# google-research/hyperbo

Measured on AMD Instinct MI355X. Metric: GP NLL+grad evals/sec at N=8192 D=16 fp64, higher is better.
Workload: dtype f64

## Files before the change

### hyperbo_amd/csrc/chol.hip

```cpp
#include "hbo_internal.h"
#include <type_traits>
#include <limits.h>
#include <string.h>

namespace {

#include "panel_dev.h"
#ifdef HBO_POTF2_TIMING
__device__ unsigned long long hbo_dbg_stamps[64];
__device__ unsigned long long hbo_dbg_wall[3 * 256];
__device__ unsigned long long hbo_dbg_trsm[3 * 128];
__device__ int hbo_dbg_trsm_panel = 36;
#define STAMP(i) do { if (threadIdx.x == 0) hbo_dbg_stamps[i] = __builtin_readcyclecounter(); } while (0)
#else
#define STAMP(i) do {} while (0)
#endif
#ifndef HBO_POTF2_WAVES
#define HBO_POTF2_WAVES 8
#endif
constexpr int POTF2_WAVES = HBO_POTF2_WAVES;
constexpr int POTF2_THREADS = 64 * POTF2_WAVES;
template <typename T>
__device__ __forceinline__ void potf2_body(const TaskDesc& t, int p, int* info_slot, unsigned char* smem) {
  typedef typename Mma<T>::acc_t acc_t;
  T* sT = reinterpret_cast<T*>(smem);
  T* sM = sT + 36 * TILE_ELEMS;
  T* sDinv = sM + TILE_ELEMS;
  const int64_t ld = t.ld;
  T* Ab = static_cast<T*>(t.A) + (int64_t)p * NB * ld + (int64_t)p * NB;
  T* Wb = static_cast<T*>(t.W) + (int64_t)p * NB * ld + (int64_t)p * NB;
  const int tid = threadIdx.x, lane = tid & 63, wave = tid >> 6;
  const int l15 = lane & 15, lq = lane >> 4;
  const int ei = (tid & 255) >> 4, ej = tid & 15;
  STAMP(0);
#ifdef HBO_POTF2_TIMING
  if (tid == 0 && blockIdx.x == 0 && p < 256) {
    hbo_dbg_wall[3 * p] = wall_clock64();
    hbo_dbg_wall[3 * p + 2] = ((unsigned long long)__builtin_amdgcn_s_getreg((20 << 0) | (0 << 6) | (31 << 11)) << 32) |
                              (unsigned)__builtin_amdgcn_s_getreg((4 << 0) | (0 << 6) | (31 << 11));
  }
#endif

  auto factor_leaf = [&](int jb, const acc_t* from_regs = nullptr) {
    T* dt = sT + tri_index(jb, jb) * TILE_ELEMS;
    acc_t acc;
    if (from_regs) acc = *from_regs;
    else {
#pragma unroll
      for (int r = 0; r < 4; ++r) acc[r] = dt[Mma<T>::crow(lane, r) * TS + l15];
    }
    const int bad = leaf_cholesky4<T>(acc, dt, sM, sDinv + jb * 16, Wb + (int64_t)(jb * 16) * ld + jb * 16, ld, lane);
    if (bad >= 0 && lane == 0) atomicMin(info_slot, p * NB + jb * 16 + bad + 1);
  };
  auto solve_tile = [&](int jb, int R) {
    T* xt = sT + tri_index(R, jb) * TILE_ELEMS;
    acc_t acc = {0, 0, 0, 0};
#pragma unroll
    for (int kk = 0; kk < 4; ++kk) acc = Mma<T>::mma(xt[l15 * TS + kk * 4 + lq], sM[l15 * TS + kk * 4 + lq], acc);
#pragma unroll
    for (int r = 0; r < 4; ++r) xt[Mma<T>::crow(lane, r) * TS + l15] = acc[r];
  };
  auto update_tile = [&](int jb, int I, int J) {
    T* ct = sT + tri_index(I, J) * TILE_ELEMS;
    const T* at = sT + tri_index(I, jb) * TILE_ELEMS;
    const T* bt = sT + tri_index(J, jb) * TILE_ELEMS;
    acc_t acc;
#pragma unroll
    for (int r = 0; r < 4; ++r) acc[r] = ct[Mma<T>::crow(lane, r) * TS + l15];
#pragma unroll
    for (int kk = 0; kk < 4; ++kk) acc = Mma<T>::mma(-at[l15 * TS + kk * 4 + lq], bt[l15 * TS + kk * 4 + lq], acc);
#pragma unroll
    for (int r = 0; r < 4; ++r) ct[Mma<T>::crow(lane, r) * TS + l15] = acc[r];
  };

  auto update_tile2 = [&](int jb, int I0, int J0, int I1, int J1) {
    T* c0 = sT + tri_index(I0, J0) * TILE_ELEMS;
    T* c1 = sT + tri_index(I1, J1) * TILE_ELEMS;
    const T* a0 = sT + tri_index(I0, jb) * TILE_ELEMS;
    const T* b0 = sT + tri_index(J0, jb) * TILE_ELEMS;
    const T* a1 = sT + tri_index(I1, jb) * TILE_ELEMS;
    const T* b1 = sT + tri_index(J1, jb) * TILE_ELEMS;
    acc_t x0, x1;
    T fa0[4], fb0[4], fa1[4], fb1[4];
#pragma unroll
    for (int r = 0; r < 4; ++r) { x0[r] = c0[Mma<T>::crow(lane, r) * TS + l15]; x1[r] = c1[Mma<T>::crow(lane, r) * TS + l15]; }
#pragma unroll
    for (int kk = 0; kk < 4; ++kk) {
      fa0[kk] = -a0[l15 * TS + kk * 4 + lq]; fb0[kk] = b0[l15 * TS + kk * 4 + lq];
      fa1[kk] = -a1[l15 * TS + kk * 4 + lq]; fb1[kk] = b1[l15 * TS + kk * 4 + lq];
    }
#pragma unroll
    for (int kk = 0; kk < 4; ++kk) { x0 = Mma<T>::mma(fa0[kk], fb0[kk], x0); x1 = Mma<T>::mma(fa1[kk], fb1[kk], x1); }
#pragma unroll
    for (int r = 0; r < 4; ++r) { c0[Mma<T>::crow(lane, r) * TS + l15] = x0[r]; c1[Mma<T>::crow(lane, r) * TS + l15] = x1[r]; }
  };

  int nleaf = 8;
  {
    const int64_t rows = (int64_t)t.n - (int64_t)p * NB;
    if (rows < NB) nleaf = rows <= 0 ? 0 : (int)((rows + 15) / 16);
    for (int jb = nleaf + wave; jb < 8; jb += POTF2_WAVES)
#pragma unroll
      for (int r = 0; r < 4; ++r) {
        const int row = Mma<T>::crow(lane, r);
        gst(Wb + (int64_t)(jb * 16 + row) * ld + jb * 16 + l15, row == l15 ? (T)1 : (T)0);
      }
    if (tid < NB && tid >= nleaf * 16) sDinv[tid] = (T)1;
  }
  const bool lead_tile0 = nleaf > 0;
  acc_t tile0 = {0, 0, 0, 0};
  if (wave == 0 && lead_tile0) {
#pragma unroll
    for (int r = 0; r < 4; ++r) {
      const int row = Mma<T>::crow(lane, r);
      const int rr = row > l15 ? row : l15, cc = row > l15 ? l15 : row;
      tile0[r] = gld(Ab + (int64_t)rr * ld + cc);
    }
  }
  constexpr int NSH = POTF2_THREADS / 256;
  const int sh = __builtin_amdgcn_readfirstlane(tid >> 8);
  T vload[36 / NSH];
  auto load_issue = [&](auto share) {
    constexpr int SH = decltype(share)::value;
    int tile = 0;
#pragma unroll
    for (int I = 0; I < 8; ++I)
#pragma unroll
      for (int J = 0; J <= I; ++J, ++tile) {
        if (tile % NSH != SH) continue;
        if (tile == 0 && lead_tile0) { vload[0] = (T)0; continue; }
        int r = ei, c = ej;
        if (I == J && ej > ei) { r = ej; c = ei; }
        vload[tile / NSH] = gld(Ab + (int64_t)(I * 16 + r) * ld + J * 16 + c);
      }
  };
  auto load_commit = [&](auto share) {
    constexpr int SH = decltype(share)::value;
#pragma unroll
    for (int k = 0; k < 36 / NSH; ++k)
      if (!(k == 0 && SH == 0 && lead_tile0)) sT[(k * NSH + SH) * TILE_ELEMS + ei * TS + ej] = vload[k];
  };
  static_assert(NSH == 1 || NSH == 2, "one or two 256-thread groups");
  if (NSH == 1 || sh == 0) load_issue(std::integral_constant<int, 0>());
  else load_issue(std::integral_constant<int, NSH - 1>());
  if (wave == 0 && lead_tile0) factor_leaf(0, &tile0);
  if (NSH == 1 || sh == 0) load_commit(std::integral_constant<int, 0>());
  else load_commit(std::integral_constant<int, NSH - 1>());
  STAMP(1);
  __syncthreads();
  STAMP(2);
  for (int jb = 0; jb < nleaf; ++jb) {
    for (int R = jb + 1 + wave; R < nleaf; R += POTF2_WAVES) solve_tile(jb, R);
    __syncthreads();
    STAMP(3 + 3 * jb);
    if (jb == nleaf - 1) break;
    {
      const int m = nleaf - 1 - jb;
      const int ntiles = m * (m + 1) / 2;
      constexpr int NH = POTF2_WAVES == 8 ? 6 : POTF2_WAVES - 1;
      const int hw = POTF2_WAVES == 8 ? (wave < 4 ? wave : wave - 1) : wave;
      const int n0 = (ntiles - 1 > 4 * NH + 1) ? (ntiles - 1 - (4 * NH + 1)) / POTF2_WAVES : 0;
      const int nshared = ntiles - n0;
      auto tile_of = [&](int tix, int& I, int& J) {
        int ii = 0;
        while ((ii + 1) * (ii + 2) / 2 <= tix) ++ii;
        I = jb + 1 + ii; J = jb + 1 + tix - ii * (ii + 1) / 2;
      };
      if (wave == 0) {
        update_tile(jb, jb + 1, jb + 1);
        factor_leaf(jb + 1);
        STAMP(4 + 3 * jb);
        for (int tix = nshared; tix < ntiles; ++tix) { int I, J; tile_of(tix, I, J); update_tile(jb, I, J); }
      } else if (!(POTF2_WAVES == 8 && wave == 4)) {
        int tix = hw;
        for (; tix + NH < nshared; tix += 2 * NH) {
          int I0, J0, I1, J1;
          tile_of(tix, I0, J0); tile_of(tix + NH, I1, J1);
          update_tile2(jb, I0, J0, I1, J1);
        }
        if (tix < nshared) { int I, J; tile_of(tix, I, J); update_tile(jb, I, J); }
      }
    }
    __syncthreads();
    STAMP(5 + 3 * jb);
  }
  STAMP(30);

  auto store_share = [&](auto share) {
    constexpr int SH = decltype(share)::value;
    int tile = 0;
#pragma unroll
    for (int I = 0; I < 8; ++I)
#pragma unroll
      for (int J = 0; J <= I; ++J, ++tile) {
        if (tile % NSH != SH) continue;
        T v = sT[tile * TILE_ELEMS + ei * TS + ej];
        if (I == J && ej > ei) v = (T)0;
        gst(Ab + (int64_t)(I * 16 + ei) * ld + J * 16 + ej, v);
      }
  };
  if (NSH == 1 || sh == 0) store_share(std::integral_constant<int, 0>());
  else store_share(std::integral_constant<int, NSH - 1>());
  STAMP(31);
  STAMP(32);
#ifdef HBO_POTF2_TIMING
  if (tid == 0 && blockIdx.x == 0 && p < 256) hbo_dbg_wall[3 * p + 1] = wall_clock64();
#endif
}
template <typename T>
__global__ __launch_bounds__(POTF2_THREADS) void potf2_kernel(const TaskDesc* tasks, int p, int* info, int* yield_flag, unsigned long long* tl) {
  extern __shared__ __attribute__((aligned(16))) unsigned char smem[];
  __builtin_amdgcn_s_setprio(3);
  const TaskDesc& t = tasks[blockIdx.x];
  if (p >= t.nblk) return;
  tl_begin(tl);
  int tok = 0;
  if (yield_flag && threadIdx.x == 0) tok = yield_enter(yield_flag);
  potf2_body<T>(t, p, info + blockIdx.x, smem);
  if (yield_flag) {
    __syncthreads();
    if (threadIdx.x == 0) yield_leave(yield_flag, tok);
  }
  tl_end(tl);
}

template <typename T>
constexpr int trsm_tile() { return sizeof(T) == 8 ? 256 : TILE_ELEMS; }
template <typename T>
__device__ __forceinline__ int trsm_at(int r, int c) { return sizeof(T) == 8 ? r * 16 + (c ^ ((r >> 1) << 1)) : r * TS + c; }
template <typename T>
constexpr int trsm_lds_bytes() { return (28 + 8 + 4) * trsm_tile<T>() * (int)sizeof(T); }
__device__ __forceinline__ int strict_index(int I, int J) { return I * (I - 1) / 2 + J; }

template <typename T, bool IDENT>
__device__ __forceinline__ void trsm_body(const TaskDesc& t, int p, int64_t row0, unsigned char* smem, bool stage) {
  typedef typename Mma<T>::acc_t acc_t;
  constexpr int TE = trsm_tile<T>();
  T* sLt = reinterpret_cast<T*>(smem);
  T* sWi = sLt + 28 * TE;
  T* sSc = sWi + 8 * TE;
  const int64_t ld = t.ld;
  const int tid = threadIdx.x, lane = tid & 63, wave = tid >> 6;
  const int l15 = lane & 15, lq = lane >> 4;
  const T* Lb = static_cast<const T*>(t.A) + (int64_t)p * NB * ld + (int64_t)p * NB;
  const T* Wb = static_cast<const T*>(t.W) + (int64_t)p * NB * ld + (int64_t)p * NB;

  const int64_t wrow0 = row0 + wave * 16;
  const int rg = IDENT ? (int)((wrow0 - (int64_t)p * NB) >> 4) : 0;
  T* Ap = IDENT ? nullptr : static_cast<T*>(t.A) + wrow0 * ld + (int64_t)p * NB;
  T* Wout = IDENT ? static_cast<T*>(t.W) + (int64_t)p * NB * ld + (int64_t)p * NB : nullptr;

  acc_t areg[8];
#pragma unroll
  for (int jb = 0; jb < 8; ++jb)
#pragma unroll
    for (int r = 0; r < 4; ++r) {
      const int row = Mma<T>::crow(lane, r);
      if (IDENT) areg[jb][r] = (rg == jb && row == l15) ? (T)1 : (T)0;
      else areg[jb][r] = gld(Ap + (int64_t)row * ld + jb * 16 + l15);
    }
  if (stage) {
    const int i = tid >> 4, j = tid & 15;
    int tile = 0;
#pragma unroll
    for (int I = 1; I < 8; ++I)
#pragma unroll
      for (int J = 0; J < I; ++J, ++tile)
        sLt[tile * TE + trsm_at<T>(i, j)] = gld(Lb + (int64_t)(I * 16 + i) * ld + J * 16 + j);
#pragma unroll
    for (int b = 0; b < 8; ++b)
      sWi[b * TE + trsm_at<T>(i, j)] = gld(Wb + (int64_t)(b * 16 + i) * ld + b * 16 + j);
  }
  if (stage) __syncthreads();

  T* sc = sSc + wave * TE;
  T xneg[8][4];
#pragma unroll
  for (int jb = 0; jb < 8; ++jb) {
    acc_t acc = areg[jb];
    acc_t acc2 = (acc_t){0, 0, 0, 0};
#pragma unroll
    for (int kb = 0; kb < 8; ++kb) {
      if (kb < jb) {
        const T* lt = sLt + strict_index(jb, kb) * TE;
#pragma unroll
        for (int kk = 0; kk < 4; ++kk) {
          const T bfrag = lt[trsm_at<T>(l15, kk * 4 + lq)];
          if (kb & 1) acc2 = Mma<T>::mma(xneg[kb][kk], bfrag, acc2);
          else acc = Mma<T>::mma(xneg[kb][kk], bfrag, acc);
        }
      }
    }
#pragma unroll
    for (int r = 0; r < 4; ++r) acc[r] += acc2[r];
    __builtin_amdgcn_wave_barrier();
#pragma unroll
    for (int r = 0; r < 4; ++r) sc[trsm_at<T>(Mma<T>::crow(lane, r), l15)] = acc[r];
    __builtin_amdgcn_wave_barrier();
    T ta[4];
#pragma unroll
    for (int kk = 0; kk < 4; ++kk) ta[kk] = sc[trsm_at<T>(l15, kk * 4 + lq)];
    acc_t x = (acc_t){0, 0, 0, 0};
    const T* wt = sWi + jb * TE;
#pragma unroll
    for (int kk = 0; kk < 4; ++kk) {
      const T bfrag = wt[trsm_at<T>(l15, kk * 4 + lq)];
      x = Mma<T>::mma(ta[kk], bfrag, x);
    }
#pragma unroll
    for (int r = 0; r < 4; ++r) {
      const int row = Mma<T>::crow(lane, r);
      if (IDENT) {
        if (rg != jb) gst(Wout + (int64_t)(jb * 16 + l15) * ld + rg * 16 + row, x[r]);
      } else {
        gst(Ap + (int64_t)row * ld + jb * 16 + l15, x[r]);
      }
    }
    if (jb < 7) {
      __builtin_amdgcn_wave_barrier();
#pragma unroll
      for (int r = 0; r < 4; ++r) sc[trsm_at<T>(Mma<T>::crow(lane, r), l15)] = x[r];
      __builtin_amdgcn_wave_barrier();
#pragma unroll
      for (int kk = 0; kk < 4; ++kk) xneg[jb][kk] = -sc[trsm_at<T>(l15, kk * 4 + lq)];
    }
  }
}
template <typename T, bool IDENT>
__global__ __launch_bounds__(256) void trsm_kernel(const TaskDesc* tasks, int p_arg, int* yield_tab, unsigned long long* tl) {
  extern __shared__ __attribute__((aligned(16))) unsigned char smem[];
  __builtin_amdgcn_s_setprio(3);
  const TaskDesc& t = tasks[blockIdx.z];
  const int p = IDENT ? p_arg + (int)blockIdx.y : p_arg;
  if (p >= t.nblk) return;
#ifdef HBO_POTF2_TIMING
  const bool dbg = !IDENT && p == hbo_dbg_trsm_panel && blockIdx.x < 128 && threadIdx.x == 0;
  if (dbg) {
    hbo_dbg_trsm[3 * blockIdx.x] = wall_clock64();
    hbo_dbg_trsm[3 * blockIdx.x + 2] = ((unsigned long long)__builtin_amdgcn_s_getreg((20 << 0) | (0 << 6) | (31 << 11)) << 32) |
                                       (unsigned)__builtin_amdgcn_s_getreg((4 << 0) | (0 << 6) | (31 << 11));
  }
#endif
  int64_t row0;
  if (IDENT) {
    row0 = (int64_t)p * NB + (int64_t)blockIdx.x * 64;
  } else {
    const int64_t first = (int64_t)(p + 1) * NB;
    const int64_t nrows = (int64_t)(t.nblk + 1) * NB - first;
    const int64_t bx = ((int64_t)blockIdx.x + 3 * (int64_t)blockIdx.z) % gridDim.x;
    if (bx * 64 >= nrows) return;
    row0 = first + bx * 64;
  }
  int tok = 0;
  tl_begin(tl);
  if (yield_tab && threadIdx.x == 0) tok = yield_enter(yield_tab);
  trsm_body<T, IDENT>(t, p, row0, smem, true);
  if (yield_tab) {
    __syncthreads();
    if (threadIdx.x == 0) yield_leave(yield_tab, tok);
  }
  tl_end(tl);
#ifdef HBO_POTF2_TIMING
  if (dbg) hbo_dbg_trsm[3 * blockIdx.x + 1] = wall_clock64();
#endif
}

template <typename T>
void set_attrs() {
  static unsigned long long seen = 0;
  if (!hbo_first_use_on_device(seen)) return;
  hipFuncSetAttribute(reinterpret_cast<const void*>(&potf2_kernel<T>),
                      hipFuncAttributeMaxDynamicSharedMemorySize, potf2_lds_bytes<T>());
  hipFuncSetAttribute(reinterpret_cast<const void*>(&trsm_kernel<T, false>),
                      hipFuncAttributeMaxDynamicSharedMemorySize, trsm_lds_bytes<T>());
  hipFuncSetAttribute(reinterpret_cast<const void*>(&trsm_kernel<T, true>),
                      hipFuncAttributeMaxDynamicSharedMemorySize, trsm_lds_bytes<T>());
}

template <typename T>
void potf2_t(const TaskDesc* tasks, int ntasks, int p, int* info, hipStream_t st, int* yield_flag, unsigned long long* tl) {
  set_attrs<T>();
  hipLaunchKernelGGL((potf2_kernel<T>), dim3(ntasks), dim3(POTF2_THREADS), potf2_lds_bytes<T>(), st, tasks, p, info,
                     yield_flag, tl);
}
template <typename T>
void trsm_t(const TaskDesc* tasks, int ntasks, int p, int max_nblk, hipStream_t st, int* yield_tab, unsigned long long* tl) {
  set_attrs<T>();
  const int nrows = (max_nblk + 1 - (p + 1)) * NB;
  if (nrows <= 0) return;
  hipLaunchKernelGGL((trsm_kernel<T, false>), dim3(nrows / 64, 1, ntasks), dim3(256), trsm_lds_bytes<T>(), st,
                     tasks, p, yield_tab, tl);
}
template <typename T>
void trtri_diag_t(const TaskDesc* tasks, int ntasks, int p_lo, int p_hi, hipStream_t st) {
  set_attrs<T>();
  if (p_hi <= p_lo) return;
  hipLaunchKernelGGL((trsm_kernel<T, true>), dim3(2, p_hi - p_lo, ntasks), dim3(256), trsm_lds_bytes<T>(), st,
                     tasks, p_lo, (int*)nullptr, (unsigned long long*)nullptr);
}

}

#ifdef HBO_POTF2_TIMING
void dbg_read_stamps(unsigned long long* host) { hipMemcpyFromSymbol(host, HIP_SYMBOL(hbo_dbg_stamps), sizeof(unsigned long long) * 64); }
extern "C" void hbo_dbg_trsm_wall(unsigned long long* host, int panel) {
  if (host) hipMemcpyFromSymbol(host, HIP_SYMBOL(hbo_dbg_trsm), sizeof(unsigned long long) * 3 * 128);
  else hipMemcpyToSymbol(HIP_SYMBOL(hbo_dbg_trsm_panel), &panel, sizeof(int));
}
extern "C" void hbo_dbg_potf2_wall(unsigned long long* host) { hipMemcpyFromSymbol(host, HIP_SYMBOL(hbo_dbg_wall), sizeof(unsigned long long) * 3 * 256); }
#endif
void launch_potf2(int dtype, const TaskDesc* tasks, int ntasks, int p, int* info, hipStream_t st, int* yield_flag, unsigned long long* tl) {
  if (dtype == HBO_F64) potf2_t<double>(tasks, ntasks, p, info, st, yield_flag, tl);
  else potf2_t<float>(tasks, ntasks, p, info, st, yield_flag, tl);
}
void launch_trsm(int dtype, const TaskDesc* tasks, int ntasks, int p, int max_nblk, hipStream_t st, int* yield_tab, unsigned long long* tl) {
  if (dtype == HBO_F64) trsm_t<double>(tasks, ntasks, p, max_nblk, st, yield_tab, tl);
  else trsm_t<float>(tasks, ntasks, p, max_nblk, st, yield_tab, tl);
}
void launch_trtri_diag(int dtype, const TaskDesc* tasks, int ntasks, int p_lo, int p_hi, hipStream_t st) {
  if (dtype == HBO_F64) trtri_diag_t<double>(tasks, ntasks, p_lo, p_hi, st);
  else trtri_diag_t<float>(tasks, ntasks, p_lo, p_hi, st);
}
```

Baseline: 93.31.

## Rework potf2 loads/stores and trsm operand layout to remove LDS transposes

The potf2 panel loads now use paired vector loads with symmetric diagonal fill. The next diagonal tile is factored straight from registers. Finished columns are written to global memory by an otherwise idle wave during the update phase, so the final store only writes the remaining tiles. The trsm kernel changes its fragment layout so solve results feed the next MMA directly from registers, which drops the per-wave scratch LDS round trips and wave barriers. It also adds a configurable wave count and occupancy hint. These changes risk subtle layout and indexing errors and add more register pressure.

```diff
diff --git a/hyperbo_amd/csrc/chol.hip b/hyperbo_amd/csrc/chol.hip
--- a/hyperbo_amd/csrc/chol.hip
+++ b/hyperbo_amd/csrc/chol.hip
@@ -73,6 +73,31 @@
     for (int r = 0; r < 4; ++r) ct[Mma<T>::crow(lane, r) * TS + l15] = acc[r];
   };
 
+  auto update_tile_regs = [&](int jb, int I, int J) -> acc_t {
+    const T* ct = sT + tri_index(I, J) * TILE_ELEMS;
+    const T* at = sT + tri_index(I, jb) * TILE_ELEMS;
+    const T* bt = sT + tri_index(J, jb) * TILE_ELEMS;
+    acc_t acc;
+#pragma unroll
+    for (int r = 0; r < 4; ++r) acc[r] = ct[Mma<T>::crow(lane, r) * TS + l15];
+#pragma unroll
+    for (int kk = 0; kk < 4; ++kk) acc = Mma<T>::mma(-at[l15 * TS + kk * 4 + lq], bt[l15 * TS + kk * 4 + lq], acc);
+    return acc;
+  };
+  auto store_column = [&](int jb, int nl) {
+#pragma unroll 2
+    for (int R = jb; R < nl; ++R) {
+      const T* tt = sT + tri_index(R, jb) * TILE_ELEMS;
+#pragma unroll
+      for (int q = 0; q < 4; ++q) {
+        const int row = 4 * q + lq;
+        T v = tt[row * TS + l15];
+        if (R == jb && l15 > row) v = (T)0;
+        gst(Ab + (int64_t)(R * 16 + row) * ld + jb * 16 + l15, v);
+      }
+    }
+  };
+
   auto update_tile2 = [&](int jb, int I0, int J0, int I1, int J1) {
     T* c0 = sT + tri_index(I0, J0) * TILE_ELEMS;
     T* c1 = sT + tri_index(I1, J1) * TILE_ELEMS;
@@ -119,33 +144,53 @@
   }
   constexpr int NSH = POTF2_THREADS / 256;
   const int sh = __builtin_amdgcn_readfirstlane(tid >> 8);
-  T vload[36 / NSH];
-  auto load_issue = [&](auto share) {
-    constexpr int SH = decltype(share)::value;
+  constexpr int NG = POTF2_THREADS / 128;
+  const int grp = __builtin_amdgcn_readfirstlane(tid >> 7);
+  const int pr = (tid & 127) >> 3, pc = (tid & 7) * 2;
+  typedef T pair_t __attribute__((ext_vector_type(2), aligned(sizeof(T))));
+  pair_t vload[(36 + NG - 1) / NG];
+  auto load_issue = [&](auto group) {
+    constexpr int G = decltype(group)::value;
     int tile = 0;
 #pragma unroll
     for (int I = 0; I < 8; ++I)
 #pragma unroll
       for (int J = 0; J <= I; ++J, ++tile) {
-        if (tile % NSH != SH) continue;
-        if (tile == 0 && lead_tile0) { vload[0] = (T)0; continue; }
-        int r = ei, c = ej;
-        if (I == J && ej > ei) { r = ej; c = ei; }
-        vload[tile / NSH] = gld(Ab + (int64_t)(I * 16 + r) * ld + J * 16 + c);
-      }
-  };
-  auto load_commit = [&](auto share) {
-    constexpr int SH = decltype(share)::value;
-#pragma unroll
-    for (int k = 0; k < 36 / NSH; ++k)
-      if (!(k == 0 && SH == 0 && lead_tile0)) sT[(k * NSH + SH) * TILE_ELEMS + ei * TS + ej] = vload[k];
+        if (tile % NG != G) continue;
+        if (tile == 0 && lead_tile0) { vload[0] = (pair_t){(T)0, (T)0}; continue; }
+        vload[tile / NG] = *(const HBO_GLOBAL pair_t*)(Ab + (int64_t)(I * 16 + pr) * ld + J * 16 + pc);
+      }
+  };
+  auto load_commit = [&](auto group) {
+    constexpr int G = decltype(group)::value;
+    int tile = 0;
+#pragma unroll
+    for (int I = 0; I < 8; ++I)
+#pragma unroll
+      for (int J = 0; J <= I; ++J, ++tile) {
+        if (tile % NG != G) continue;
+        if (tile == 0 && lead_tile0) continue;
+        T* tt = sT + tile * TILE_ELEMS;
+        const pair_t v = vload[tile / NG];
+        if (I == J) {
+          if (pc <= pr) { tt[pr * TS + pc] = v[0]; tt[pc * TS + pr] = v[0]; }
+          if (pc + 1 <= pr) { tt[pr * TS + pc + 1] = v[1]; tt[(pc + 1) * TS + pr] = v[1]; }
+        } else {
+          tt[pr * TS + pc] = v[0]; tt[pr * TS + pc + 1] = v[1];
+        }
+      }
   };
   static_assert(NSH == 1 || NSH == 2, "one or two 256-thread groups");
-  if (NSH == 1 || sh == 0) load_issue(std::integral_constant<int, 0>());
-  else load_issue(std::integral_constant<int, NSH - 1>());
+  static_assert(NG == 2 || NG == 4, "two or four 128-thread groups");
+  auto by_group = [&](auto f) {
+    if (grp == 0) f(std::integral_constant<int, 0>());
+    else if (grp == 1) f(std::integral_constant<int, 1>());
+    else if (NG == 4 && grp == 2) f(std::integral_constant<int, 2 % NG>());
+    else f(std::integral_constant<int, NG - 1>());
+  };
+  by_group(load_issue);
   if (wave == 0 && lead_tile0) factor_leaf(0, &tile0);
-  if (NSH == 1 || sh == 0) load_commit(std::integral_constant<int, 0>());
-  else load_commit(std::integral_constant<int, NSH - 1>());
+  by_group(load_commit);
   STAMP(1);
   __syncthreads();
   STAMP(2);
@@ -167,11 +212,14 @@
         I = jb + 1 + ii; J = jb + 1 + tix - ii * (ii + 1) / 2;
       };
       if (wave == 0) {
-        update_tile(jb, jb + 1, jb + 1);
-        factor_leaf(jb + 1);
+        const acc_t next_diag = update_tile_regs(jb, jb + 1, jb + 1);
+        factor_leaf(jb + 1, &next_diag);
         STAMP(4 + 3 * jb);
         for (int tix = nshared; tix < ntiles; ++tix) { int I, J; tile_of(tix, I, J); update_tile(jb, I, J); }
-      } else if (!(POTF2_WAVES == 8 && wave == 4)) {
+      } else if (POTF2_WAVES == 8 && wave == 4) {
+        store_column(jb, nleaf);
+      } else {
+        if (POTF2_WAVES != 8 && wave == POTF2_WAVES - 1) store_column(jb, nleaf);
         int tix = hw;
         for (; tix + NH < nshared; tix += 2 * NH) {
           int I0, J0, I1, J1;
@@ -194,12 +242,15 @@
 #pragma unroll
       for (int J = 0; J <= I; ++J, ++tile) {
         if (tile % NSH != SH) continue;
+        if (J < nleaf - 1 && I < nleaf) continue;
         T v = sT[tile * TILE_ELEMS + ei * TS + ej];
         if (I == J && ej > ei) v = (T)0;
         gst(Ab + (int64_t)(I * 16 + ei) * ld + J * 16 + ej, v);
       }
   };
-  if (NSH == 1 || sh == 0) store_share(std::integral_constant<int, 0>());
+  if (nleaf == 8) {
+    if (tid < 256) gst(Ab + (int64_t)(7 * 16 + ei) * ld + 7 * 16 + ej, ej > ei ? (T)0 : sT[35 * TILE_ELEMS + ei * TS + ej]);
+  } else if (NSH == 1 || sh == 0) store_share(std::integral_constant<int, 0>());
   else store_share(std::integral_constant<int, NSH - 1>());
   STAMP(31);
   STAMP(32);
@@ -224,12 +275,25 @@
   tl_end(tl);
 }
 
-template <typename T>
-constexpr int trsm_tile() { return sizeof(T) == 8 ? 256 : TILE_ELEMS; }
-template <typename T>
-__device__ __forceinline__ int trsm_at(int r, int c) { return sizeof(T) == 8 ? r * 16 + (c ^ ((r >> 1) << 1)) : r * TS + c; }
-template <typename T>
-constexpr int trsm_lds_bytes() { return (28 + 8 + 4) * trsm_tile<T>() * (int)sizeof(T); }
+#ifndef HBO_TRSM_WAVES
+#define HBO_TRSM_WAVES 4
+#endif
+constexpr int TRSM_WAVES = HBO_TRSM_WAVES;
+constexpr int TRSM_THREADS = 64 * TRSM_WAVES;
+constexpr int TRSM_ROWS = 16 * TRSM_WAVES;
+static_assert(TRSM_WAVES == 4 || TRSM_WAVES == 8, "one or two 256-thread groups; NB rows are a whole number of workgroups");
+template <typename T>
+constexpr int trsm_tile() { return 256; }
+template <typename T>
+__device__ __forceinline__ int trsm_kcol(int lq, int r) { return sizeof(T) == 8 ? 2 * lq + (r & 1) + 8 * (r >> 1) : lq + 4 * r; }
+template <typename T>
+__device__ __forceinline__ int trsm_arow(int i) { return sizeof(T) == 8 ? 2 * (i & 3) + ((i >> 2) & 1) + (i & 8) : (i >> 2) + 4 * (i & 3); }
+template <typename T>
+__device__ __forceinline__ int trsm_at(int r, int c) {
+  return sizeof(T) == 8 ? r * 16 + (c ^ ((r & 12) | ((r & 1) << 1) | ((r >> 1) & 1))) : r * 16 + (c ^ r);
+}
+template <typename T>
+constexpr int trsm_lds_bytes() { return (28 + 8) * trsm_tile<T>() * (int)sizeof(T); }
 __device__ __forceinline__ int strict_index(int I, int J) { return I * (I - 1) / 2 + J; }
 
 template <typename T, bool IDENT>
@@ -238,96 +302,87 @@
   constexpr int TE = trsm_tile<T>();
   T* sLt = reinterpret_cast<T*>(smem);
   T* sWi = sLt + 28 * TE;
-  T* sSc = sWi + 8 * TE;
   const int64_t ld = t.ld;
   const int tid = threadIdx.x, lane = tid & 63, wave = tid >> 6;
   const int l15 = lane & 15, lq = lane >> 4;
+  const int ar = trsm_arow<T>(l15);
   const T* Lb = static_cast<const T*>(t.A) + (int64_t)p * NB * ld + (int64_t)p * NB;
   const T* Wb = static_cast<const T*>(t.W) + (int64_t)p * NB * ld + (int64_t)p * NB;
 
   const int64_t wrow0 = row0 + wave * 16;
   const int rg = IDENT ? (int)((wrow0 - (int64_t)p * NB) >> 4) : 0;
-  T* Ap = IDENT ? nullptr : static_cast<T*>(t.A) + wrow0 * ld + (int64_t)p * NB;
+  T* Ap = IDENT ? nullptr : static_cast<T*>(t.A) + (wrow0 + l15) * ld + (int64_t)p * NB;
   T* Wout = IDENT ? static_cast<T*>(t.W) + (int64_t)p * NB * ld + (int64_t)p * NB : nullptr;
 
-  acc_t areg[8];
+  acc_t y[8];
 #pragma unroll
   for (int jb = 0; jb < 8; ++jb)
 #pragma unroll
     for (int r = 0; r < 4; ++r) {
-      const int row = Mma<T>::crow(lane, r);
-      if (IDENT) areg[jb][r] = (rg == jb && row == l15) ? (T)1 : (T)0;
-      else areg[jb][r] = gld(Ap + (int64_t)row * ld + jb * 16 + l15);
+      const int k = trsm_kcol<T>(lq, r);
+      if (IDENT) y[jb][r] = (rg == jb && k == l15) ? (T)1 : (T)0;
+      else y[jb][r] = gld(Ap + jb * 16 + k);
     }
   if (stage) {
-    const int i = tid >> 4, j = tid & 15;
-    int tile = 0;
-#pragma unroll
-    for (int I = 1; I < 8; ++I)
-#pragma unroll
-      for (int J = 0; J < I; ++J, ++tile)
-        sLt[tile * TE + trsm_at<T>(i, j)] = gld(Lb + (int64_t)(I * 16 + i) * ld + J * 16 + j);
-#pragma unroll
-    for (int b = 0; b < 8; ++b)
-      sWi[b * TE + trsm_at<T>(i, j)] = gld(Wb + (int64_t)(b * 16 + i) * ld + b * 16 + j);
-  }
-  if (stage) __syncthreads();
-
-  T* sc = sSc + wave * TE;
-  T xneg[8][4];
+    constexpr int NSH = TRSM_THREADS / 256;
+    const int i = (tid & 255) >> 4, j = tid & 15;
+    auto stage_share = [&](auto share) {
+      constexpr int SH = decltype(share)::value;
+      T v[36 / NSH];
+      int tile = 0;
+#pragma unroll
+      for (int I = 1; I < 8; ++I)
+#pragma unroll
+        for (int J = 0; J < I; ++J, ++tile)
+          if (tile % NSH == SH) v[tile / NSH] = gld(Lb + (int64_t)(I * 16 + i) * ld + J * 16 + j);
+#pragma unroll
+      for (int b = 0; b < 8; ++b)
+        if ((28 + b) % NSH == SH) v[(28 + b) / NSH] = gld(Wb + (int64_t)(b * 16 + i) * ld + b * 16 + j);
+#pragma unroll
+      for (int q = 0; q < 36 / NSH; ++q) sLt[(q * NSH + SH) * TE + trsm_at<T>(i, j)] = v[q];
+    };
+    if (NSH == 1 || __builtin_amdgcn_readfirstlane(tid >> 8) == 0) stage_share(std::integral_constant<int, 0>());
+    else stage_share(std::integral_constant<int, NSH - 1>());
+    __syncthreads();
+  }
+
 #pragma unroll
   for (int jb = 0; jb < 8; ++jb) {
-    acc_t acc = areg[jb];
+    acc_t acc = y[jb];
     acc_t acc2 = (acc_t){0, 0, 0, 0};
 #pragma unroll
     for (int kb = 0; kb < 8; ++kb) {
       if (kb < jb) {
         const T* lt = sLt + strict_index(jb, kb) * TE;
 #pragma unroll
-        for (int kk = 0; kk < 4; ++kk) {
-          const T bfrag = lt[trsm_at<T>(l15, kk * 4 + lq)];
-          if (kb & 1) acc2 = Mma<T>::mma(xneg[kb][kk], bfrag, acc2);
-          else acc = Mma<T>::mma(xneg[kb][kk], bfrag, acc);
+        for (int r = 0; r < 4; ++r) {
+          const T afrag = lt[trsm_at<T>(ar, trsm_kcol<T>(lq, r))];
+          if (kb & 1) acc2 = Mma<T>::mma(afrag, y[kb][r], acc2);
+          else acc = Mma<T>::mma(afrag, y[kb][r], acc);
         }
       }
     }
 #pragma unroll
     for (int r = 0; r < 4; ++r) acc[r] += acc2[r];
-    __builtin_amdgcn_wave_barrier();
-#pragma unroll
-    for (int r = 0; r < 4; ++r) sc[trsm_at<T>(Mma<T>::crow(lane, r), l15)] = acc[r];
-    __builtin_amdgcn_wave_barrier();
-    T ta[4];
-#pragma unroll
-    for (int kk = 0; kk < 4; ++kk) ta[kk] = sc[trsm_at<T>(l15, kk * 4 + lq)];
     acc_t x = (acc_t){0, 0, 0, 0};
     const T* wt = sWi + jb * TE;
 #pragma unroll
-    for (int kk = 0; kk < 4; ++kk) {
-      const T bfrag = wt[trsm_at<T>(l15, kk * 4 + lq)];
-      x = Mma<T>::mma(ta[kk], bfrag, x);
-    }
+    for (int r = 0; r < 4; ++r) x = Mma<T>::mma(wt[trsm_at<T>(ar, trsm_kcol<T>(lq, r))], acc[r], x);
 #pragma unroll
     for (int r = 0; r < 4; ++r) {
-      const int row = Mma<T>::crow(lane, r);
+      const int k = trsm_kcol<T>(lq, r);
       if (IDENT) {
-        if (rg != jb) gst(Wout + (int64_t)(jb * 16 + l15) * ld + rg * 16 + row, x[r]);
+        if (rg != jb) gst(Wout + (int64_t)(jb * 16 + k) * ld + rg * 16 + l15, x[r]);
       } else {
-        gst(Ap + (int64_t)row * ld + jb * 16 + l15, x[r]);
-      }
-    }
-    if (jb < 7) {
-      __builtin_amdgcn_wave_barrier();
-#pragma unroll
-      for (int r = 0; r < 4; ++r) sc[trsm_at<T>(Mma<T>::crow(lane, r), l15)] = x[r];
-      __builtin_amdgcn_wave_barrier();
-#pragma unroll
-      for (int kk = 0; kk < 4; ++kk) xneg[jb][kk] = -sc[trsm_at<T>(l15, kk * 4 + lq)];
-    }
+        gst(Ap + jb * 16 + k, x[r]);
+      }
+    }
+#pragma unroll
+    for (int r = 0; r < 4; ++r) y[jb][r] = -x[r];
   }
 }
 template <typename T, bool IDENT>
-__global__ __launch_bounds__(256) void trsm_kernel(const TaskDesc* tasks, int p_arg, int* yield_tab, unsigned long long* tl) {
+__global__ __launch_bounds__(TRSM_THREADS, 4) void trsm_kernel(const TaskDesc* tasks, int p_arg, int* yield_tab, unsigned long long* tl) {
   extern __shared__ __attribute__((aligned(16))) unsigned char smem[];
   __builtin_amdgcn_s_setprio(3);
   const TaskDesc& t = tasks[blockIdx.z];
@@ -343,13 +398,13 @@
 #endif
   int64_t row0;
   if (IDENT) {
-    row0 = (int64_t)p * NB + (int64_t)blockIdx.x * 64;
+    row0 = (int64_t)p * NB + (int64_t)blockIdx.x * TRSM_ROWS;
   } else {
     const int64_t first = (int64_t)(p + 1) * NB;
     const int64_t nrows = (int64_t)(t.nblk + 1) * NB - first;
     const int64_t bx = ((int64_t)blockIdx.x + 3 * (int64_t)blockIdx.z) % gridDim.x;
-    if (bx * 64 >= nrows) return;
-    row0 = first + bx * 64;
+    if (bx * TRSM_ROWS >= nrows) return;
+    row0 = first + bx * TRSM_ROWS;
   }
   int tok = 0;
   tl_begin(tl);
@@ -388,14 +443,14 @@
   set_attrs<T>();
   const int nrows = (max_nblk + 1 - (p + 1)) * NB;
   if (nrows <= 0) return;
-  hipLaunchKernelGGL((trsm_kernel<T, false>), dim3(nrows / 64, 1, ntasks), dim3(256), trsm_lds_bytes<T>(), st,
+  hipLaunchKernelGGL((trsm_kernel<T, false>), dim3(nrows / TRSM_ROWS, 1, ntasks), dim3(TRSM_THREADS), trsm_lds_bytes<T>(), st,
                      tasks, p, yield_tab, tl);
 }
 template <typename T>
 void trtri_diag_t(const TaskDesc* tasks, int ntasks, int p_lo, int p_hi, hipStream_t st) {
   set_attrs<T>();
   if (p_hi <= p_lo) return;
-  hipLaunchKernelGGL((trsm_kernel<T, true>), dim3(2, p_hi - p_lo, ntasks), dim3(256), trsm_lds_bytes<T>(), st,
+  hipLaunchKernelGGL((trsm_kernel<T, true>), dim3(NB / TRSM_ROWS, p_hi - p_lo, ntasks), dim3(TRSM_THREADS), trsm_lds_bytes<T>(), st,
                      tasks, p_lo, (int*)nullptr, (unsigned long long*)nullptr);
 }
 
```

New measurement: 93.34 (median of 3 runs). Within noise of the previous version (+0.0%).
